# KhanhNguyen4999/Speech-Enhancement-CLSKD

Hardware: AMD Instinct MI355X
Metric: frames/sec/GPU DCCRN-CLSKD fwd+loss @16k 4s; SI-SNR parity ±0.01 dB (higher is better)
Workload: dtype bf16; 1 GPU; C2: DCCRN-CLSKD fwd+loss (teacher 3.67M + student 0.23M params, ReviewKD enc+dec, 14 SPKD Grams, MRSTFT); global_batch=16, per_gpu_batch=16, clip_samples=64000, frames_per_clip=643, parallelism=dp1, abf_reinit=step

## Files before the change

include/clskd.h:

```cpp
#ifndef CLSKD_H
#define CLSKD_H

#include <stdint.h>

#ifdef __cplusplus
extern "C" {
#endif

typedef enum {
  CLSKD_OK = 0,
  CLSKD_E_SHAPE = -1,
  CLSKD_E_DTYPE = -2,
  CLSKD_E_HIP = -3,
  CLSKD_E_ARG = -4
} clskd_status;

typedef enum { CLSKD_F32 = 0, CLSKD_BF16 = 1, CLSKD_F16 = 2, CLSKD_F32X3 = 3 } clskd_compute;

const char* clskd_last_error(void);
int clskd_version(void);

int clskd_set_knob(const char* name, int32_t value);
int clskd_get_knob(const char* name, int32_t* value);
int clskd_experiments_build(void);
// ... 43 lines not shown
  const struct clskd_bn_fold_s* bn_fold;
} clskd_conv_desc;

#define CLSKD_BN_FOLD_REPL 8
typedef struct clskd_bn_fold_s {
  int64_t* acc;
  uint32_t* ticket;
  int32_t finalize;
  int32_t C;
  int32_t c_off;
  int32_t n_updates;
  int64_t count;
  const float* gamma;
  const float* beta;
  float eps, momentum;
  float* running_mean;
  float* running_var;
  float* scale;
  float* shift;
  float* mean_out;
  float* var_out;
} clskd_bn_fold;

int64_t clskd_bn_fold_state_size(int32_t C);
int clskd_abf_bn1_fold(const float* s, int32_t B, int32_t F, int32_t T, int64_t sB, int64_t sF,
                       int64_t sT, int32_t cin, const float* w1, const clskd_bn_fold* fold,
                       int32_t nblk, void* stream);
int32_t clskd_conv_fold_capable(const clskd_conv_desc* d);

#define CLSKD_WLAYOUT_NK 0
#define CLSKD_WLAYOUT_DIRECT 1

int clskd_conv2d_fwd(const clskd_conv_desc* d, void* stream);
const char* clskd_conv_last_kernel(void);
const void* clskd_conv_last_kernel_fn(void);
int32_t clskd_conv_last_stream_k(void);
int clskd_stream_prepare(void* stream);
int clskd_capture_scope_begin(void* const* streams, int32_t nstreams, void** scope);
int clskd_capture_scope_end(void* scope);
int clskd_capture_scope_free(void* scope);
int clskd_conv_direct_np(int32_t N);
int clskd_conv_direct_ok(int32_t N, int32_t K);

int clskd_bn_stats_partial(const void* x, int64_t rows, int32_t C, double* partial,
                           int32_t nblk, int32_t dtype, void* stream);
int clskd_bn_compact(const double* partial, int32_t nblk, int32_t C, int32_t group, double* out,
                     void* stream);
int clskd_bn_finalize(double* partial, int32_t nblk, int64_t rows, int32_t C,
                      const float* gamma, const float* beta, float eps,
                      float* running_mean, float* running_var, float momentum,
                      int32_t n_updates, float* scale, float* shift, float* mean_out,
                      float* var_out, void* stream);
int clskd_bn_eval_coeffs(const float* running_mean, const float* running_var,
                         const float* gamma, const float* beta, float eps, int32_t C,
                         float* scale, float* shift, void* stream);
int clskd_bn_apply(const void* x, void* y, int64_t rows, int32_t C, const float* scale,
                   const float* shift, const float* alpha, int32_t dtype, void* stream);
int clskd_bn_apply_reim(const void* x, void* y, int64_t rows, int32_t C, const float* scale,
                        const float* shift, const float* alpha_re_im, int32_t dtype,
                        void* stream);
int32_t clskd_bn_partial_blocks(int64_t rows, int32_t C);

int clskd_lstm_recurrent(const float* gx, int64_t gx_ws, int64_t gx_seq, int64_t gx_t,
                         const float* whh, int32_t nws, int32_t nseq, int32_t T, int32_t H,
                         float* out, int64_t o_ws, int64_t o_seq, int64_t o_t, void* stream);
int clskd_lstm_pre_capable(int32_t H);
// ... 285 lines not shown
```

speech-enhancement-clskd_amd/clskd/_lib.py:

```python
import ctypes as C
import os

import torch

_HERE = os.path.dirname(os.path.abspath(__file__))
_LIB_ENV = os.environ.get("CLSKD_LIB", "")
LIB_PATH = os.path.join(_HERE, "libclskd_hip_exp.so" if _LIB_ENV == "exp"
                        else (os.path.basename(_LIB_ENV) if _LIB_ENV.endswith(".so")
                              else "libclskd_hip.so"))

MAX_SEGS = 4
F32, BF16, F16 = 0, 1, 2
F32X3 = 3
WLAYOUT_NK, WLAYOUT_DIRECT = 0, 1


class Seg(C.Structure):
    _fields_ = [("ptr", C.c_void_p), ("sB", C.c_int64), ("sF", C.c_int64), ("sT", C.c_int64),
                ("F", C.c_int32), ("T", C.c_int32)]


class KtabEntry(C.Structure):
    _fields_ = [("off", C.c_int32), ("dF", C.c_int16), ("dT", C.c_int16)]


class ConvDesc(C.Structure):
    _fields_ = [("B", C.c_int32), ("Fo", C.c_int32), ("To", C.c_int32), ("N", C.c_int32),
                ("K", C.c_int32), ("stride_f", C.c_int32), ("stride_t", C.c_int32),
                ("nseg", C.c_int32), ("seg", Seg * MAX_SEGS), ("ktab", C.c_void_p),
                ("kseg", C.c_void_p), ("vec4", C.c_int32), ("weight", C.c_void_p),
                ("bias", C.c_void_p), ("out", C.c_void_p), ("oB", C.c_int64), ("oF", C.c_int64),
                ("oT", C.c_int64), ("oNhi", C.c_int64), ("oNlo", C.c_int64), ("nlo", C.c_int32),
                ("of_mul", C.c_int32), ("of_add", C.c_int32), ("compute", C.c_int32),
                ("in_dtype", C.c_int32), ("out_dtype", C.c_int32), ("stats", C.c_void_p),
                ("kvec", C.c_int32), ("wlayout", C.c_int32), ("ntaps", C.c_int32),
                ("ctot", C.c_int32), ("seg_c", C.c_int32 * MAX_SEGS), ("tap_df", C.c_int16 * 16),
                ("tap_dt", C.c_int16 * 16), ("accumulate", C.c_int32), ("reserved_", C.c_int32),
                ("bn_fold", C.c_void_p)]


BN_FOLD_REPL = 8


class BnFold(C.Structure):
    _fields_ = [("acc", C.c_void_p), ("ticket", C.c_void_p), ("finalize", C.c_int32),
                ("C", C.c_int32), ("c_off", C.c_int32), ("n_updates", C.c_int32),
                ("count", C.c_int64), ("gamma", C.c_void_p), ("beta", C.c_void_p),
                ("eps", C.c_float), ("momentum", C.c_float), ("running_mean", C.c_void_p),
                ("running_var", C.c_void_p), ("scale", C.c_void_p), ("shift", C.c_void_p),
                ("mean_out", C.c_void_p), ("var_out", C.c_void_p)]


class GramJob(C.Structure):
    _fields_ = [("ptr", C.c_void_p), ("sB", C.c_int64), ("P", C.c_int64), ("Ctot", C.c_int32),
                ("c0", C.c_int32), ("Cs", C.c_int32), ("chunk", C.c_int32),
                ("first_slab", C.c_int32), ("nslab", C.c_int32), ("dtype", C.c_int32),
                ("reserved", C.c_int32), ("scale", C.c_void_p), ("shift", C.c_void_p),
                ("alpha", C.c_void_p), ("out", C.c_void_p)]


class DrawJob(C.Structure):
    _fields_ = [("param", C.c_void_p), ("packed", C.c_void_p), ("numel", C.c_int64),
                ("Cin", C.c_int32), ("ntap", C.c_int32), ("Kp", C.c_int32),
                ("packed_dtype", C.c_int32), ("bound", C.c_float), ("stream_id", C.c_int32)]


class GramBwdJob(C.Structure):
    _fields_ = [("ptr", C.c_void_p), ("sB", C.c_int64), ("P", C.c_int64), ("Ctot", C.c_int32),
                ("c0", C.c_int32), ("Cs", C.c_int32), ("dtype", C.c_int32), ("scale", C.c_void_p),
                ("shift", C.c_void_p), ("coef", C.c_void_p), ("out", C.c_void_p),
                ("o_sB", C.c_int64), ("o_Ctot", C.c_int32), ("o_c0", C.c_int32),
# ... 34 lines not shown


assert C.sizeof(KtabEntry) == 8
assert C.sizeof(DrawJob) == 48
assert C.sizeof(GramJob) == 88

_p, _i32, _i64, _f32 = C.c_void_p, C.c_int32, C.c_int64, C.c_float

GATHER_JOBS_MAX = 48


class GatherJob(C.Structure):
    _fields_ = [("src", C.c_void_p), ("idx", C.c_void_p), ("sgn", C.c_void_p), ("out", C.c_void_p),
                ("n", C.c_int64), ("J", C.c_int32), ("accumulate", C.c_int32)]

SIGNATURES = {
    "clskd_last_error": (C.c_char_p, []),
    "clskd_conv_last_kernel": (C.c_char_p, []),
    "clskd_conv_last_kernel_fn": (_p, []),
    "clskd_conv_last_stream_k": (_i32, []),
    "clskd_exec_launch_ahead": (_i32, [_p, _p, C.c_uint32, _p]),
    "clskd_stream_prepare": (_i32, [_p]),
    "clskd_capture_scope_begin": (_i32, [_p, _i32, _p]),
    "clskd_exec_census": (_i32, [_p, _p, _i32, _p, _p, _p]),
    "clskd_kernel_name": (_i32, [_p, _p, _i32]),
    "clskd_capture_scope_end": (_i32, [_p]),
    "clskd_capture_scope_free": (_i32, [_p]),
    "clskd_version": (_i32, []),
    "clskd_set_knob": (_i32, [C.c_char_p, _i32]),
    "clskd_get_knob": (_i32, [C.c_char_p, C.POINTER(C.c_int32)]),
    "clskd_experiments_build": (_i32, []),
    "clskd_conv2d_fwd": (_i32, [C.POINTER(ConvDesc), _p]),
    "clskd_conv_fold_capable": (_i32, [C.POINTER(ConvDesc)]),
    "clskd_bn_fold_state_size": (_i64, [_i32]),
    "clskd_abf_bn1_fold": (_i32, [_p, _i32, _i32, _i32, _i64, _i64, _i64, _i32, _p, _p, _i32, _p]),
    "clskd_conv_direct_np": (_i32, [_i32]),
    "clskd_conv_direct_ok": (_i32, [_i32, _i32]),
    "clskd_bn_partial_blocks": (_i32, [_i64, _i32]),
    "clskd_bn_stats_partial": (_i32, [_p, _i64, _i32, _p, _i32, _i32, _p]),
    "clskd_bn_compact": (_i32, [_p, _i32, _i32, _i32, _p, _p]),
    "clskd_bn_finalize": (_i32, [_p, _i32, _i64, _i32, _p, _p, _f32, _p, _p, _f32, _i32, _p, _p,
                                 _p, _p, _p]),
    "clskd_bn_eval_coeffs": (_i32, [_p, _p, _p, _p, _f32, _i32, _p, _p, _p]),
    "clskd_bn_apply": (_i32, [_p, _p, _i64, _i32, _p, _p, _p, _i32, _p]),
    "clskd_bn_apply_reim": (_i32, [_p, _p, _i64, _i32, _p, _p, _p, _i32, _p]),
    "clskd_mask_bdt": (_i32, [_p, _i32, _p, _i32, _i32, _i32, _p, _i32, _p]),
    "clskd_lstm_recurrent": (_i32, [_p, _i64, _i64, _i64, _p, _i32, _i32, _i32, _i32, _p, _i64,
                                    _i64, _i64, _p]),
    "clskd_lstm_recurrent_pre": (_i32, [_p, _i64, _i64, _i64, _p, _i32, _i32, _i32, _i32, _p, _i64,
                                        _i64, _i64, _p, _p]),
    "clskd_lstm_pre_capable": (_i32, [_i32]),
    "clskd_complex_combine": (_i32, [_p, _p, _p, _p, _p, _p, _i64, _p]),
    "clskd_complex_combine_dt": (_i32, [_p, _p, _p, _p, _p, _p, _i64, _i32, _p]),
    "clskd_lstm_cell": (_i32, [_p, _i64, _i64, _p, _i32, _i32, _i32, _p, _p, _i64, _i64, _p, _i64,
                               _i64, _p]),
    "clskd_frame_pad": (_i32, [_p, _i64, _i32, _i32, _i32, _i32, _i32, _p, _p]),
    "clskd_spec_bftc": (_i32, [_p, _i32, _i32, _i32, _i32, _i32, _i32, _p, _p]),
    "clskd_mask_e": (_i32, [_p, _i32, _p, _i32, _i32, _i32, _p, _i32, _p, _p, _p]),
    "clskd_ola": (_i32, [_p, _p, _i32, _i32, _i32, _i32, _i32, _i32, _i32, _p, _p]),
    "clskd_abf_fuse": (_i32, [_p, _p, _i32, _i32, _i32, _i32, _i32, _p, _p, _p, _p, _p, _i32,
                              _p]),
    "clskd_abf_moment_blocks": (_i32, [_i64, _i32]),
    "clskd_abf_bn1_partials": (_i32, [_p, _i32, _i32, _i32, _i64, _i64, _i64, _i32, _p, _p, _i32,
                                      _p]),
    "clskd_abf_conv1_fuse": (_i32, [_p, _i32, _i32, _i32, _i64, _i64, _i64, _i32, _p, _p, _p, _p,
                                    _i32, _i32, _p, _p, _p, _p, _i32, _p]),
# ... 150 lines not shown
```

speech-enhancement-clskd_amd/clskd/build.py:

```python
import concurrent.futures as cf
import os
import subprocess

HERE = os.path.dirname(os.path.abspath(__file__))
CSRC = os.path.join(os.path.dirname(HERE), "csrc")
OUT = os.path.join(HERE, "libclskd_hip.so")
OUT_EXP = os.path.join(HERE, "libclskd_hip_exp.so")
OBJDIR = os.path.join(os.path.dirname(HERE), "build", "obj")
OBJDIR_EXP = os.path.join(os.path.dirname(HERE), "build", "obj_exp")
HIPCC = os.environ.get("HIPCC", "/opt/rocm/bin/hipcc")
ARCH = "gfx950"
SOURCES = ["capi.cpp", "conv_igemm.hip", "conv_bf16.hip", "conv_halo.hip", "conv_halo32.hip", "conv_gemm8.hip", "conv_split.hip", "conv_direct.hip", "conv_pointwise.hip", "norm.hip", "lstm.hip", "loss.hip", "redraw.hip", "grad.hip", "wgrad_x3.hip", "norm_bwd.hip", "abf.hip", "metrics.hip", "exec.cpp", "stream_hop.hip", "stream_hop_mini.hip"]
EXPERIMENT_SOURCES = ["conv_halow.hip"]
FLAGS = ["-O3", "-fPIC", "-std=c++17", f"--offload-arch={ARCH}", "-Wall", "-Wno-unused-function"]


def _newer(src_files, target):
    if not os.path.exists(target):
        return True
    t = os.path.getmtime(target)
    return any(os.path.getmtime(s) > t for s in src_files)


def build(verbose=False, force=False, experiments=None):
    if experiments is None:
        experiments = os.environ.get("CLSKD_EXPERIMENTS") == "1"
    objdir, out = (OBJDIR_EXP, OUT_EXP) if experiments else (OBJDIR, OUT)
    flags = FLAGS + (["-DCLSKD_EXPERIMENTS"] if experiments else [])
    os.makedirs(objdir, exist_ok=True)
    headers = [os.path.join(CSRC, f) for f in os.listdir(CSRC) if f.endswith(".h")]
    headers.append(os.path.join(os.path.dirname(os.path.dirname(HERE)), "include", "clskd.h"))
    objs = []
    jobs = []
    for s in SOURCES + (EXPERIMENT_SOURCES if experiments else []):
        src = os.path.join(CSRC, s)
        obj = os.path.join(objdir, s + ".o")
        objs.append(obj)
        if force or _newer([src] + headers, obj):
            lang = ["-x", "hip"] if s.endswith(".hip") else []
            jobs.append([HIPCC] + flags + lang + ["-c", src, "-o", obj])
    with cf.ThreadPoolExecutor(max_workers=min(8, max(1, len(jobs)))) as ex:
        for cmd, res in zip(jobs, ex.map(lambda c: subprocess.run(c, capture_output=True, text=True), jobs)):
            if res.returncode != 0:
                raise RuntimeError(f"hipcc failed: {' '.join(cmd)}\n{res.stdout}\n{res.stderr}")
            if verbose and res.stderr.strip():
# ... 12 lines not shown
```

speech-enhancement-clskd_amd/csrc/capi.cpp:

```cpp
#include <stdarg.h>
#include <stdio.h>
#include <stdlib.h>

#include <atomic>
#include <mutex>

#include "common.h"

namespace clskd {
static thread_local char g_err[512] = "";
void set_error(const char* fmt, ...) {
  va_list ap;
  va_start(ap, fmt);
  vsnprintf(g_err, sizeof(g_err), fmt, ap);
  va_end(ap);
}
static thread_local char g_kernel[160] = "";
void note_kernel(const char* fmt, ...) {
  va_list ap;
  va_start(ap, fmt);
  vsnprintf(g_kernel, sizeof(g_kernel), fmt, ap);
  va_end(ap);
}

// ... 1 lines not shown
void note_kernel_fn(const void* fn) { g_kernel_fn = fn; }

struct KnobDef {
  const char* name;
  int dflt;
  bool product;
};
static const KnobDef kKnobs[KNOB_COUNT] = {
    {"CLSKD_G8", 1, false},          {"CLSKD_G8_GRID", 0, true},      {"CLSKD_HALO_GRID", 0, false},
    {"CLSKD_LSTM_NKS", 4, false},    {"CLSKD_LSTM_NKS32", 1, true},   {"CLSKD_WGRAD_WG", 4096, false},
    {"CLSKD_NO_HALO", 0, false},     {"CLSKD_BF16_WAVES", 8, false},  {"CLSKD_BF16_STAGES", 3, false},
    {"CLSKD_BF16_TILE", 0, false},   {"CLSKD_NO_POINTWISE", 0, false},
    {"CLSKD_ABF_MOMENT_DIV", 1, false}, {"CLSKD_F32_WAVES", 4, false}, {"CLSKD_EXEC_GATE", 0, false},
    {"CLSKD_NO_HALO32", 0, true},
    {"CLSKD_HALO32_SPLIT", 0, true}, {"CLSKD_HALO32_MIN_N", 32, true}, {"CLSKD_G8_KORDER", 1, false},
    {"CLSKD_G8_PP", 0, false},
    {"CLSKD_F32_SPLIT", 0, true},
    {"CLSKD_LSTM_PRIO", 0, true},
    {"CLSKD_SPLIT_BK", 0, true},
    {"CLSKD_HALOW", 0, false},
    {"CLSKD_SPLIT_GRID", 0, true},
    {"CLSKD_G8_TA", 1, true},
    {"CLSKD_G8_SK", 1, true},
    {"CLSKD_SPLIT_PD", 1, true},
    {"CLSKD_SPLIT_OCC", 1, true},
    {"CLSKD_WGRAD_DEPTH", 0, true},
    {"CLSKD_LSTM_BWD_WAVE", 1, true},
    {"CLSKD_SPLIT_NS2", 1, true},
    {"CLSKD_BN_PFOLD", 1, true},
    {"CLSKD_LSTM_PRE", 1, true},
    {"CLSKD_ABF_BWD_BLOCKS", 2048, false},
    {"CLSKD_WGRAD_XCD", 1, true},
    {"CLSKD_LSTM_BWD_PIN", 1, true},
    {"CLSKD_LSTM128_TDIV", 0, false},
    {"CLSKD_LSTM32_TDIV", 0, false}, {"CLSKD_BF16_DEBUG_MODE", 0, false}, {"CLSKD_SKIP", 0, false},
    {"CLSKD_H32_DEBUG_MODE", 0, false},
};
#ifdef CLSKD_EXPERIMENTS
static constexpr bool kAllKnobs = true;
#else
static constexpr bool kAllKnobs = false;
#endif
static std::atomic<int> g_knob[KNOB_COUNT];
static std::once_flag g_knob_once;

static void init_knobs() {
  for (int i = 0; i < KNOB_COUNT; ++i) {
    const char* e = (kAllKnobs || kKnobs[i].product) ? getenv(kKnobs[i].name) : nullptr;
    g_knob[i].store(e && *e ? atoi(e) : kKnobs[i].dflt, std::memory_order_relaxed);
  }
}

int knob(KnobId k) {
  std::call_once(g_knob_once, init_knobs);
  return g_knob[k].load(std::memory_order_relaxed);
}

static int knob_index(const char* name) {
  if (!name) return -1;
  for (int i = 0; i < KNOB_COUNT; ++i)
    if (strcmp(name, kKnobs[i].name) == 0) return i;
  return -1;
}

bool skip_kernel(int bit) {
#ifdef CLSKD_EXPERIMENTS
// ... 54 lines not shown
```

speech-enhancement-clskd_amd/csrc/common.h:

```cpp
#pragma once
#include <hip/hip_runtime.h>
#include <stdint.h>
#include <stdio.h>
#include <string.h>

#include "../../include/clskd.h"

namespace clskd {

void set_error(const char* fmt, ...);
void note_kernel(const char* fmt, ...);
void note_kernel_fn(const void* fn);
enum KnobId {
  KNOB_G8, KNOB_G8_GRID, KNOB_HALO_GRID, KNOB_LSTM_NKS, KNOB_LSTM_NKS32,
  KNOB_WGRAD_WG, KNOB_NO_HALO, KNOB_BF16_WAVES, KNOB_BF16_STAGES, KNOB_BF16_TILE,
  KNOB_NO_POINTWISE, KNOB_ABF_MOMENT_DIV, KNOB_F32_WAVES, KNOB_EXEC_GATE,
  KNOB_NO_HALO32, KNOB_HALO32_SPLIT, KNOB_HALO32_MIN_N, KNOB_G8_KORDER, KNOB_G8_PP, KNOB_F32_SPLIT, KNOB_LSTM_PRIO, KNOB_SPLIT_BK, KNOB_HALOW, KNOB_SPLIT_GRID, KNOB_G8_TA, KNOB_G8_SK, KNOB_SPLIT_PD, KNOB_SPLIT_OCC, KNOB_WGRAD_DEPTH, KNOB_LSTM_BWD_WAVE, KNOB_SPLIT_NS2, KNOB_BN_PFOLD, KNOB_LSTM_PRE, KNOB_ABF_BWD_BLOCKS, KNOB_WGRAD_XCD, KNOB_LSTM_BWD_PIN,
  KNOB_LSTM128_TDIV, KNOB_LSTM32_TDIV, KNOB_BF16_DEBUG_MODE, KNOB_SKIP, KNOB_H32_DEBUG_MODE,
  KNOB_COUNT
};
int knob(KnobId k);
int fold_partials(double* part, int nblk, int E, int bit, hipStream_t st);
int experiment_guard(const char* what, int value);
enum SkipBit {
  SKIP_BN_FINALIZE = 1, SKIP_BN_APPLY = 2, SKIP_CONV_F32 = 4, SKIP_LSTM = 8, SKIP_ABF = 16,
  SKIP_GRAM = 32, SKIP_CONV_LOWP = 64, SKIP_CONV_DIRECT = 128, SKIP_LSTM_PRE = 256, SKIP_LSTM_BWD = 512
};
bool skip_kernel(int bit);
template <typename T> inline const char* type_name();
template <> inline const char* type_name<float>() { return "float"; }
template <> inline const char* type_name<__bf16>() { return "bf16"; }
template <> inline const char* type_name<_Float16>() { return "f16"; }
template <typename T> constexpr int lowp_code() { return sizeof(T) == 4 ? CLSKD_F32 : CLSKD_BF16; }
template <> constexpr int lowp_code<_Float16>() { return CLSKD_F16; }
inline bool is_lowp(int dt) { return dt == CLSKD_BF16 || dt == CLSKD_F16; }

#define CLSKD_CHECK_ARG(cond, ...)                 \
  do {                                             \
    if (!(cond)) {                                 \
      ::clskd::set_error(__VA_ARGS__);             \
      return CLSKD_E_ARG;                          \
    }                                              \
  } while (0)

#define CLSKD_CHECK_SHAPE(cond, ...)               \
  do {                                             \
    if (!(cond)) {                                 \
      ::clskd::set_error(__VA_ARGS__);             \
      return CLSKD_E_SHAPE;                        \
    }                                              \
// ... 135 lines not shown
```

speech-enhancement-clskd_amd/csrc/conv_igemm.hip:

```cpp
#include <stdlib.h>

#include "common.h"

namespace clskd {

constexpr int BK = 16;

struct ConvArgs {
  clskd_conv_desc d;
  int kt_taps, kt_cpt;
};

__device__ __forceinline__ int swz(int row, int chunk) { return chunk ^ ((row >> 2) & 3); }

template <typename T>
__device__ __forceinline__ T sel4(int s, T a0, T a1, T a2, T a3) {
  const T lo = (s & 1) ? a1 : a0;
  const T hi = (s & 1) ? a3 : a2;
  return (s & 2) ? hi : lo;
}

template <typename OutT>
__device__ __forceinline__ void store_val(OutT* p, float v) { *p = (OutT)v; }

// ... 254 lines not shown
      d.stats[(blk * d.N + n) * 2] = S;
      d.stats[(blk * d.N + n) * 2 + 1] = Q;
    }
  }

  OutT* outp = reinterpret_cast<OutT*>(d.out);
#pragma unroll
  for (int t = 0; t < NT; ++t) {
    const int n = n0 + t * 32 + (lane & 31);
    if (n >= d.N) continue;
    const int64_t coff = (int64_t)(n / d.nlo) * d.oNhi + (int64_t)(n % d.nlo) * d.oNlo;
#pragma unroll
    for (int r = 0; r < 16; ++r) {
      const int row = wave * 32 + (r & 3) + 8 * (r >> 2) + 4 * h;
      const int64_t ro = out_row[row];
      if (ro >= 0) {
        float v = acc[t][r];
        if constexpr (sizeof(OutT) == 4) {
          if (d.accumulate) v += outp[ro + coff];
        }
        store_val<OutT>(outp + ro + coff, v);
      }
    }
  }
}

int launch_conv_bf16(const clskd_conv_desc& d, hipStream_t st);

int launch_conv_direct(const clskd_conv_desc& d, hipStream_t st);

int launch_conv_pointwise(const clskd_conv_desc& d, hipStream_t st, bool* launched);
int launch_conv_halo_f32(const clskd_conv_desc& d, hipStream_t st, bool* launched);
int launch_conv_split3(const clskd_conv_desc& d, hipStream_t st, bool* launched, bool force);

}

using namespace clskd;

namespace clskd {
bool conv_halo_takes(const clskd_conv_desc& d);
bool conv_halo_f32_takes(const clskd_conv_desc& d);
bool conv_gemm8_takes(const clskd_conv_desc& d);
#ifdef CLSKD_EXPERIMENTS
bool conv_halow_takes(const clskd_conv_desc& d);
#endif
bool conv_pointwise_takes(const clskd_conv_desc& d);
bool conv_split3_takes(const clskd_conv_desc& d, bool force);
}

static bool fold_capable(const clskd_conv_desc& dd) {
  if (dd.wlayout == CLSKD_WLAYOUT_DIRECT || dd.accumulate) return false;
  if (is_lowp(dd.compute)) {
    if (conv_halo_takes(dd)) return true;
#ifdef CLSKD_EXPERIMENTS
    if (conv_halow_takes(dd)) return true;
#endif
    return conv_gemm8_takes(dd) && dd.N <= 256;
  }
  const bool split = dd.compute == CLSKD_F32X3;
  clskd_conv_desc d = dd;
  d.compute = CLSKD_F32;
  if (conv_pointwise_takes(d)) return false;
  if (conv_split3_takes(d, split)) return true;
  return knob(KNOB_NO_HALO32) != 1 && conv_halo_f32_takes(d);
}

extern "C" int32_t clskd_conv_fold_capable(const clskd_conv_desc* dp) {
  if (!dp) return 0;
  return fold_capable(*dp) ? 1 : 0;
}

extern "C" int64_t clskd_bn_fold_state_size(int32_t C) {
  return C > 0 ? (int64_t)CLSKD_BN_FOLD_REPL * C * 6 : 0;
}

extern "C" int clskd_conv2d_fwd(const clskd_conv_desc* dp, void* stream) {
  CLSKD_CHECK_ARG(dp != nullptr, "conv2d: null descriptor");
  CLSKD_CHECK_ARG(dp->compute == CLSKD_F32 || dp->compute == CLSKD_BF16 || dp->compute == CLSKD_F16 ||
                      dp->compute == CLSKD_F32X3,
                  "conv2d: unknown compute %d", dp->compute);
  CLSKD_CHECK_ARG(dp->compute != CLSKD_F32X3 || dp->in_dtype == CLSKD_F32,
                  "conv2d: split products (CLSKD_F32X3) take fp32 segments");
  const bool want_split = dp->compute == CLSKD_F32X3;
  clskd_conv_desc dcopy = *dp;
  if (want_split) dcopy.compute = CLSKD_F32;
  const clskd_conv_desc& d = dcopy;
  CLSKD_CHECK_SHAPE(d.B > 0 && d.Fo > 0 && d.To > 0 && d.N > 0 && d.K > 0, "conv2d: empty shape");
  if (const clskd_bn_fold* f = d.bn_fold) {
    CLSKD_CHECK_ARG(!d.stats, "conv2d: bn_fold and stats are exclusive");
    CLSKD_CHECK_ARG(f->acc && f->ticket && f->scale && f->shift, "conv2d: bn_fold null pointer");
    CLSKD_CHECK_SHAPE(f->C > 0 && f->c_off >= 0 && f->c_off + d.N <= f->C && f->count > 0,
                      "conv2d: bn_fold channels [%d, +%d) outside C=%d", f->c_off, d.N, f->C);
    CLSKD_CHECK_ARG(fold_capable(*dp), "conv2d: N=%d K=%d dispatches to a kernel without the folded "
                    "BatchNorm finalize (clskd_conv_fold_capable)", d.N, d.K);
  }
// ... 27 lines not shown
  }
  const int64_t M = (int64_t)d.B * d.Fo * d.To;
  CLSKD_CHECK_SHAPE(M < (int64_t)INT32_MAX * 64, "conv2d: too many rows");
  hipStream_t st = as_stream(stream);
  CLSKD_CHECK_SHAPE(d.kvec == 0 || d.kvec == 1 || d.kvec == 2 || d.kvec == 4 || d.kvec == 8,
                    "conv2d: kvec=%d", d.kvec);
  CLSKD_CHECK_ARG(d.wlayout == CLSKD_WLAYOUT_NK || d.wlayout == CLSKD_WLAYOUT_DIRECT,
                  "conv2d: wlayout=%d", d.wlayout);
  CLSKD_CHECK_ARG(!d.accumulate || ((d.compute == CLSKD_F32 || d.compute == CLSKD_BF16) &&
                                     d.out_dtype == CLSKD_F32),
                  "conv2d: accumulate needs fp32 or bf16 compute and an fp32 output (the fp32 "
                  "engines, the direct kernel, the bf16 LDS-DMA engine)");
  if (d.wlayout == CLSKD_WLAYOUT_DIRECT) {
    if (skip_kernel(SKIP_CONV_DIRECT)) return CLSKD_OK;
    const int rc = launch_conv_direct(d, st);
    if (rc != CLSKD_OK) return rc;
    CLSKD_LAUNCH_CHECK("conv2d_direct");
    return CLSKD_OK;
  }
  if (lowp) {
    if (skip_kernel(SKIP_CONV_LOWP)) return CLSKD_OK;
    const int rc = launch_conv_bf16(d, st);
    if (rc != CLSKD_OK) return rc;
    CLSKD_LAUNCH_CHECK("conv2d_bf16");
    return CLSKD_OK;
  }
  if (skip_kernel(SKIP_CONV_F32)) return CLSKD_OK;
  {
    bool launched = false;
    const int rc = launch_conv_pointwise(d, st, &launched);
    if (rc != CLSKD_OK) return rc;
    if (launched) {
      CLSKD_LAUNCH_CHECK("conv2d_pointwise");
      return CLSKD_OK;
    }
  }
  {
    bool launched = false;
    const int rc = launch_conv_split3(d, st, &launched, want_split);
    if (rc != CLSKD_OK) return rc;
    if (launched) {
      CLSKD_LAUNCH_CHECK("conv2d_split3");
      return CLSKD_OK;
    }
  }
  if (knob(KNOB_NO_HALO32) != 1) {
    bool launched = false;
    const int rc = launch_conv_halo_f32(d, st, &launched);
    if (rc != CLSKD_OK) return rc;
    if (launched) {
      CLSKD_LAUNCH_CHECK("conv2d_halo_f32");
      return CLSKD_OK;
    }
  }
  ConvArgs a{d, 1, d.K / BK};
  if (knob(KNOB_G8_KORDER) != 0 && d.vec4 && d.ntaps > 1 && d.ctot % BK == 0 &&
      (int64_t)d.ntaps * d.ctot == d.K) {
    a.kt_taps = d.ntaps;
    a.kt_cpt = d.ctot / BK;
  }
  const size_t ctab_bytes = (size_t)(d.K / 4) * 8;
  CLSKD_CHECK_SHAPE(!d.vec4 || ctab_bytes <= 32 * 1024, "conv2d(f32): K=%d too long for the chunk table", d.K);
  const int nw = knob(KNOB_F32_WAVES) == 8 ? 8 : 4;
#define LAUNCH(BN_, V_, O_, NW_)                                                             \
  do {                                                                                       \
    hipLaunchKernelGGL((conv_igemm_f32<BN_, V_, O_, NW_>),                                    \
// ... 28 lines not shown
```

Measured before the change: 2.007 million frames/s.

## Add halo-tiled split-bf16 (3-pass) MFMA conv kernel for F32X3 convolutions

```diff
diff --git a/include/clskd.h b/include/clskd.h
--- a/include/clskd.h
+++ b/include/clskd.h
@@ -99,6 +99,21 @@
 #define CLSKD_WLAYOUT_DIRECT 1
 
 int clskd_conv2d_fwd(const clskd_conv_desc* d, void* stream);
+
+typedef struct {
+  int32_t launches, col_halves;
+  int32_t cw;
+  int32_t tile_f, tile_t;
+  int32_t nfb, ntb, ntiles;
+  int32_t halo_f, halo_t;
+  int32_t nchunk, nstep;
+  int32_t grid;
+  int32_t reserved_;
+  int64_t lds_bytes;
+  int64_t seg_min_off[CLSKD_MAX_SEGS];
+  int64_t seg_max_off[CLSKD_MAX_SEGS];
+} clskd_halo_split_info;
+int clskd_conv_halo_split_plan(const clskd_conv_desc* d, clskd_halo_split_info* info);
 const char* clskd_conv_last_kernel(void);
 const void* clskd_conv_last_kernel_fn(void);
 int32_t clskd_conv_last_stream_k(void);
diff --git a/speech-enhancement-clskd_amd/clskd/_lib.py b/speech-enhancement-clskd_amd/clskd/_lib.py
--- a/speech-enhancement-clskd_amd/clskd/_lib.py
+++ b/speech-enhancement-clskd_amd/clskd/_lib.py
@@ -37,6 +37,15 @@
                 ("ctot", C.c_int32), ("seg_c", C.c_int32 * MAX_SEGS), ("tap_df", C.c_int16 * 16),
                 ("tap_dt", C.c_int16 * 16), ("accumulate", C.c_int32), ("reserved_", C.c_int32),
                 ("bn_fold", C.c_void_p)]
+
+
+class HaloSplitInfo(C.Structure):
+    _fields_ = [("launches", C.c_int32), ("col_halves", C.c_int32), ("cw", C.c_int32), ("tile_f", C.c_int32),
+                ("tile_t", C.c_int32), ("nfb", C.c_int32), ("ntb", C.c_int32),
+                ("ntiles", C.c_int32), ("halo_f", C.c_int32), ("halo_t", C.c_int32),
+                ("nchunk", C.c_int32), ("nstep", C.c_int32), ("grid", C.c_int32), ("reserved_", C.c_int32),
+                ("lds_bytes", C.c_int64), ("seg_min_off", C.c_int64 * MAX_SEGS),
+                ("seg_max_off", C.c_int64 * MAX_SEGS)]
 
 
 BN_FOLD_REPL = 8
@@ -137,6 +146,7 @@
     "clskd_experiments_build": (_i32, []),
     "clskd_conv2d_fwd": (_i32, [C.POINTER(ConvDesc), _p]),
     "clskd_conv_fold_capable": (_i32, [C.POINTER(ConvDesc)]),
+    "clskd_conv_halo_split_plan": (_i32, [C.POINTER(ConvDesc), C.POINTER(HaloSplitInfo)]),
     "clskd_bn_fold_state_size": (_i64, [_i32]),
     "clskd_abf_bn1_fold": (_i32, [_p, _i32, _i32, _i32, _i64, _i64, _i64, _i32, _p, _p, _i32, _p]),
     "clskd_conv_direct_np": (_i32, [_i32]),
diff --git a/speech-enhancement-clskd_amd/clskd/build.py b/speech-enhancement-clskd_amd/clskd/build.py
--- a/speech-enhancement-clskd_amd/clskd/build.py
+++ b/speech-enhancement-clskd_amd/clskd/build.py
@@ -10,7 +10,7 @@
 OBJDIR_EXP = os.path.join(os.path.dirname(HERE), "build", "obj_exp")
 HIPCC = os.environ.get("HIPCC", "/opt/rocm/bin/hipcc")
 ARCH = "gfx950"
-SOURCES = ["capi.cpp", "conv_igemm.hip", "conv_bf16.hip", "conv_halo.hip", "conv_halo32.hip", "conv_gemm8.hip", "conv_split.hip", "conv_direct.hip", "conv_pointwise.hip", "norm.hip", "lstm.hip", "loss.hip", "redraw.hip", "grad.hip", "wgrad_x3.hip", "norm_bwd.hip", "abf.hip", "metrics.hip", "exec.cpp", "stream_hop.hip", "stream_hop_mini.hip"]
+SOURCES = ["capi.cpp", "conv_igemm.hip", "conv_bf16.hip", "conv_halo.hip", "conv_halo32.hip", "conv_gemm8.hip", "conv_split.hip", "conv_halo_split.hip", "conv_direct.hip", "conv_pointwise.hip", "norm.hip", "lstm.hip", "loss.hip", "redraw.hip", "grad.hip", "wgrad_x3.hip", "norm_bwd.hip", "abf.hip", "metrics.hip", "exec.cpp", "stream_hop.hip", "stream_hop_mini.hip"]
 EXPERIMENT_SOURCES = ["conv_halow.hip"]
 FLAGS = ["-O3", "-fPIC", "-std=c++17", f"--offload-arch={ARCH}", "-Wall", "-Wno-unused-function"]
 
diff --git a/speech-enhancement-clskd_amd/csrc/capi.cpp b/speech-enhancement-clskd_amd/csrc/capi.cpp
--- a/speech-enhancement-clskd_amd/csrc/capi.cpp
+++ b/speech-enhancement-clskd_amd/csrc/capi.cpp
@@ -57,6 +57,8 @@
     {"CLSKD_ABF_BWD_BLOCKS", 2048, false},
     {"CLSKD_WGRAD_XCD", 1, true},
     {"CLSKD_LSTM_BWD_PIN", 1, true},
+    {"CLSKD_HALO_SPLIT", 1, true},
+    {"CLSKD_HALO_SPLIT_GRID", 0, true},
     {"CLSKD_LSTM128_TDIV", 0, false},
     {"CLSKD_LSTM32_TDIV", 0, false}, {"CLSKD_BF16_DEBUG_MODE", 0, false}, {"CLSKD_SKIP", 0, false},
     {"CLSKD_H32_DEBUG_MODE", 0, false},
diff --git a/speech-enhancement-clskd_amd/csrc/common.h b/speech-enhancement-clskd_amd/csrc/common.h
--- a/speech-enhancement-clskd_amd/csrc/common.h
+++ b/speech-enhancement-clskd_amd/csrc/common.h
@@ -16,6 +16,7 @@
   KNOB_WGRAD_WG, KNOB_NO_HALO, KNOB_BF16_WAVES, KNOB_BF16_STAGES, KNOB_BF16_TILE,
   KNOB_NO_POINTWISE, KNOB_ABF_MOMENT_DIV, KNOB_F32_WAVES, KNOB_EXEC_GATE,
   KNOB_NO_HALO32, KNOB_HALO32_SPLIT, KNOB_HALO32_MIN_N, KNOB_G8_KORDER, KNOB_G8_PP, KNOB_F32_SPLIT, KNOB_LSTM_PRIO, KNOB_SPLIT_BK, KNOB_HALOW, KNOB_SPLIT_GRID, KNOB_G8_TA, KNOB_G8_SK, KNOB_SPLIT_PD, KNOB_SPLIT_OCC, KNOB_WGRAD_DEPTH, KNOB_LSTM_BWD_WAVE, KNOB_SPLIT_NS2, KNOB_BN_PFOLD, KNOB_LSTM_PRE, KNOB_ABF_BWD_BLOCKS, KNOB_WGRAD_XCD, KNOB_LSTM_BWD_PIN,
+  KNOB_HALO_SPLIT, KNOB_HALO_SPLIT_GRID,
   KNOB_LSTM128_TDIV, KNOB_LSTM32_TDIV, KNOB_BF16_DEBUG_MODE, KNOB_SKIP, KNOB_H32_DEBUG_MODE,
   KNOB_COUNT
 };
diff --git a/speech-enhancement-clskd_amd/csrc/conv_halo_split.hip b/speech-enhancement-clskd_amd/csrc/conv_halo_split.hip
--- /dev/null
+++ b/speech-enhancement-clskd_amd/csrc/conv_halo_split.hip
@@ -0,0 +1,580 @@
+#include <stdlib.h>
+
+#include "bnfold.h"
+#include "common.h"
+
+namespace clskd {
+
+__device__ __attribute__((aligned(256))) unsigned char g_hs3_sink[4096];
+
+typedef __attribute__((address_space(1))) float gfloat_hs3;
+
+namespace hs3 {
+typedef short s16x8 __attribute__((ext_vector_type(8)));
+typedef short s16x4 __attribute__((ext_vector_type(4)));
+constexpr int NW = 8;
+constexpr int NTH = NW * 64;
+constexpr int MAXU = 6;
+constexpr int MAXCH = 64;
+constexpr int MAXSTEP = 16;
+
+__device__ __forceinline__ void split4(const f32x4 v, s16x4& hi, s16x4& lo) {
+  bf16x4 h, l;
+#pragma unroll
+  for (int i = 0; i < 4; ++i) {
+    h[i] = (__bf16)v[i];
+    l[i] = (__bf16)(v[i] - (float)h[i]);
+  }
+  hi = __builtin_bit_cast(s16x4, h);
+  lo = __builtin_bit_cast(s16x4, l);
+}
+
+__host__ __device__ inline int plane_off(int cw, int p, int q) {
+  return cw == 16 ? p * 32 + ((((q >> 1) ^ (p >> 3)) & 1) << 4) + (q & 1) * 8 : p * 16 + (q & 1) * 8;
+}
+}
+
+struct HaloSplitArgs {
+  clskd_conv_desc d;
+  int32_t nchunk;
+  int32_t chunk_seg[hs3::MAXCH];
+  int32_t chunk_c0[hs3::MAXCH];
+  int32_t chunk_kofs[hs3::MAXCH];
+  int32_t cw, tw;
+  int32_t dfmin, dtmin;
+  int32_t HF, HT, NPIX;
+  int32_t NU;
+  int32_t plane_bytes;
+  int32_t nstep;
+  int32_t step_pix[2][hs3::MAXSTEP];
+  int32_t step_oct[2][hs3::MAXSTEP];
+  int32_t koct;
+  int32_t nfb, ntb, ntiles;
+  int32_t nblk128;
+  int32_t stats_ld;
+  int32_t nhalf;
+  BnFoldArgs f;
+};
+
+template <int NB, int CW, int NSTEP>
+__global__ __launch_bounds__(512) void conv_halo_split3_kernel(const HaloSplitArgs a) {
+  using namespace hs3;
+  const clskd_conv_desc& d = a.d;
+  constexpr int NBW = NB * 32;
+  constexpr int QP = CW / 4;
+  constexpr int NACC = NB == 1 ? 3 : 1;
+  extern __shared__ __attribute__((aligned(16))) unsigned char smem[];
+  const int plane_bytes = a.plane_bytes;
+  unsigned char* hbuf = smem;
+  unsigned char* wl = smem + 4 * plane_bytes;
+  const int wplane = (a.koct + 1) * NBW * 16;
+  int4* ctA = reinterpret_cast<int4*>(wl + 2 * wplane);
+  int4* ctB = ctA + MAXCH;
+
+  const int tid = threadIdx.x;
+  const int lane = tid & 63;
+  const int wave = __builtin_amdgcn_readfirstlane(tid >> 6);
+  const int l32 = lane & 31, h = lane >> 5;
+  const int nhalf = a.nhalf;
+  const int half = nhalf == 2 ? (int)(blockIdx.x & 1) : 0;
+  const int wgi = blockIdx.x / nhalf, nwg = gridDim.x / nhalf;
+  const int n0 = half * 32;
+  const int N = nhalf == 2 ? min(32, d.N - n0) : d.N;
+
+  {
+    const int64_t K = d.K;
+    const float* wg = reinterpret_cast<const float*>(d.weight) + n0 * K;
+    const int total = a.koct * NBW * 2;
+    constexpr int WB = 8;
+    const int kq2 = a.koct * 2;
+    for (int base = tid; base < total; base += NTH * WB) {
+      f32x4 v[WB];
+#pragma unroll
+      for (int j = 0; j < WB; ++j) {
+        const int idx = base + j * NTH;
+        const int n = idx / kq2, kq = idx - n * kq2;
+        v[j] = (idx < total && n < N) ? *reinterpret_cast<const f32x4*>(wg + n * K + kq * 4)
+                                      : f32x4{0.f, 0.f, 0.f, 0.f};
+      }
+#pragma unroll
+      for (int j = 0; j < WB; ++j) {
+        const int idx = base + j * NTH;
+        if (idx < total) {
+          const int n = idx / kq2, kq = idx - n * kq2;
+          s16x4 hi, lo;
+          split4(v[j], hi, lo);
+          const int off = ((kq >> 1) * NBW + n) * 16 + (kq & 1) * 8;
+          *reinterpret_cast<s16x4*>(wl + off) = hi;
+          *reinterpret_cast<s16x4*>(wl + wplane + off) = lo;
+        }
+      }
+    }
+    for (int i = tid; i < NBW * 4; i += NTH) {
+      const int pl = i / (NBW * 2), piece = i - pl * NBW * 2;
+      *reinterpret_cast<int2*>(wl + pl * wplane + a.koct * NBW * 16 + piece * 8) = make_int2(0, 0);
+    }
+  }
+  if (tid < a.nchunk) {
+    const clskd_seg& S = d.seg[a.chunk_seg[tid]];
+    const uint64_t base = (uint64_t)(uintptr_t)(S.ptr + a.chunk_c0[tid]);
+    ctA[tid] = make_int4((int)(unsigned)base, (int)(unsigned)(base >> 32), (int)S.sF, (int)S.sT);
+    ctB[tid] = make_int4((int)S.sB, S.F, S.T, a.chunk_kofs[tid]);
+  }
+  if (d.stats) {
+    for (int64_t s = (int64_t)blockIdx.x + gridDim.x; s < a.nblk128; s += gridDim.x)
+      for (int i = tid; i < d.N * 2; i += NTH) d.stats[s * a.stats_ld * 2 + i] = 0.0;
+    if (nhalf == 2)
+      for (int i = tid; i < (d.N - N) * 2; i += NTH)
+        d.stats[((int64_t)blockIdx.x * a.stats_ld + (half ? 0 : 32)) * 2 + i] = 0.0;
+  }
+  float bcol[NB];
+  int64_t coff[NB];
+#pragma unroll
+  for (int nb = 0; nb < NB; ++nb) {
+    const int n = nb * 32 + l32;
+    const int ng = n0 + n;
+    bcol[nb] = (d.bias && n < N) ? d.bias[ng] : 0.f;
+    coff[nb] = n < N ? (int64_t)(ng / d.nlo) * d.oNhi + (int64_t)(ng % d.nlo) * d.oNlo : -1;
+  }
+  const int nchunk = a.nchunk, ntb = a.ntb, nfb = a.nfb, NU = a.NU;
+  const int tw = a.tw, FT = NW / tw, TT = 32 * tw;
+  const int Fo = d.Fo, To = d.To, sfr = d.stride_f;
+  const int dfmin = a.dfmin, dtmin = a.dtmin;
+  const int64_t oB = d.oB, oF = d.oF, oT = d.oT;
+  const int of_mul = d.of_mul, of_add = d.of_add;
+  gfloat_hs3* const outp = reinterpret_cast<gfloat_hs3*>((uintptr_t)d.out);
+  int ug[MAXU], uo[MAXU];
+  {
+    const int HT = a.HT, NPIX = a.NPIX;
+#pragma unroll
+    for (int i = 0; i < MAXU; ++i) {
+      const int u = tid + i * NTH;
+      const int p = u / QP, q = u % QP;
+      const bool ok = i < NU && p < NPIX;
+      const int pp = ok ? p : 0;
+      const int hf = pp / HT, ht = pp - hf * HT;
+      ug[i] = hf | (ht << 8) | (q << 16) | ((ok ? 1 : 0) << 20);
+      uo[i] = plane_off(CW, pp, q);
+    }
+  }
+  const int frow = wave / tw, tblk = wave - frow * tw;
+  int sa[NSTEP];
+  unsigned sb[NSTEP];
+  {
+    const int prow0 = frow * sfr * a.HT + tblk * 32 + l32;
+#pragma unroll
+    for (int s = 0; s < NSTEP; ++s) {
+      const int p = prow0 + (h ? a.step_pix[1][s] : a.step_pix[0][s]);
+      const int oct = h ? a.step_oct[1][s] : a.step_oct[0][s];
+      sa[s] = CW == 16 ? p * 32 + (((h ^ (p >> 3)) & 1) << 4) : p * 16;
+      sb[s] = oct < 0 ? (0x80000000u | (unsigned)((a.koct * NBW + l32) * 16))
+                      : (unsigned)((oct * NBW + l32) * 16);
+    }
+  }
+  __syncthreads();
+
+  const int per = (a.ntiles + nwg - 1) / nwg;
+  const int tile_begin = wgi * per;
+  const int ntile_blk = max(0, min(a.ntiles, tile_begin + per) - tile_begin);
+
+  struct Cur { int b, fb, tb; };
+  auto cur_of = [&](int tile) {
+    Cur c;
+    c.tb = tile % ntb;
+    const int r = tile / ntb;
+    c.fb = r % nfb;
+    c.b = r / nfb;
+    return c;
+  };
+  auto advance = [&](Cur& c) {
+    if (++c.tb == ntb) {
+      c.tb = 0;
+      if (++c.fb == nfb) { c.fb = 0; ++c.b; }
+    }
+  };
+
+  f32x4 ra[MAXU];
+  auto load_chunk = [&](const Cur& c, int ch) {
+    const int4 ea = ctA[ch];
+    const int4 eb = ctB[ch];
+    const float* base = reinterpret_cast<const float*>(((uint64_t)(unsigned)ea.y << 32) | (unsigned)ea.x) +
+                        (int64_t)c.b * eb.x;
+    const int fi_lo = c.fb * FT * sfr + dfmin, ti_lo = c.tb * TT + dtmin;
+#pragma unroll
+    for (int i = 0; i < MAXU; ++i) {
+      if (i < NU) {
+        const int g = ug[i];
+        const int fi = fi_lo + (g & 0xff), ti = ti_lo + ((g >> 8) & 0xff);
+        f32x4 v = {0.f, 0.f, 0.f, 0.f};
+        if (((g >> 20) & 1) && (unsigned)fi < (unsigned)eb.y && (unsigned)ti < (unsigned)eb.z)
+          v = *reinterpret_cast<const f32x4*>(base + (int64_t)fi * ea.z + (int64_t)ti * ea.w +
+                                              ((g >> 16) & 3) * 4);
+        ra[i] = v;
+      }
+    }
+  };
+  auto store_chunk = [&](int buf) {
+    unsigned char* hb = hbuf + buf * 2 * plane_bytes;
+#pragma unroll
+    for (int i = 0; i < MAXU; ++i) {
+      if (i < NU && ((ug[i] >> 20) & 1)) {
+        s16x4 hi, lo;
+        split4(ra[i], hi, lo);
+        *reinterpret_cast<s16x4*>(hb + uo[i]) = hi;
+        *reinterpret_cast<s16x4*>(hb + plane_bytes + uo[i]) = lo;
+      }
+    }
+  };
+
+  f32x16 acc[NACC][NB];
+  double st_s[NB], st_q[NB];
+#pragma unroll
+  for (int nb = 0; nb < NB; ++nb) st_s[nb] = st_q[nb] = 0.0;
+
+  const int total = ntile_blk * nchunk;
+  Cur cur = cur_of(tile_begin), nxt = cur;
+  int nxt_ch = 0;
+  auto step_next = [&]() {
+    if (++nxt_ch == nchunk) { nxt_ch = 0; advance(nxt); }
+  };
+  if (total > 0) {
+    load_chunk(nxt, nxt_ch);
+    step_next();
+    store_chunk(0);
+    if (total > 1) {
+      load_chunk(nxt, nxt_ch);
+      step_next();
+    }
+  }
+  __syncthreads();
+
+  int it = 0;
+  for (int ti = 0; ti < ntile_blk; ++ti) {
+#pragma unroll
+    for (int q = 0; q < NACC; ++q)
+#pragma unroll
+      for (int nb = 0; nb < NB; ++nb)
+#pragma unroll
+        for (int r = 0; r < 16; ++r) acc[q][nb][r] = q == 0 ? bcol[nb] : 0.f;
+    for (int ch = 0; ch < nchunk; ++ch, ++it) {
+      const unsigned char* hb = hbuf + (it & 1) * 2 * plane_bytes;
+      const unsigned kofsb = (unsigned)((ctB[ch].w >> 3) * NBW * 16);
+#pragma unroll
+      for (int s = 0; s < NSTEP; ++s) {
+        const s16x8 ahi = *reinterpret_cast<const s16x8*>(hb + sa[s]);
+        const s16x8 alo = *reinterpret_cast<const s16x8*>(hb + plane_bytes + sa[s]);
+        const unsigned bo = (sb[s] & 0x7fffffffu) + ((sb[s] >> 31) ? 0u : kofsb);
+        s16x8 bhi[NB], blo[NB];
+#pragma unroll
+        for (int nb = 0; nb < NB; ++nb) {
+          bhi[nb] = *reinterpret_cast<const s16x8*>(wl + bo + nb * 512);
+          blo[nb] = *reinterpret_cast<const s16x8*>(wl + wplane + bo + nb * 512);
+        }
+        if constexpr (NB == 1) {
+          acc[0][0] = mfma16<__bf16>(ahi, bhi[0], acc[0][0]);
+          acc[1][0] = mfma16<__bf16>(alo, bhi[0], acc[1][0]);
+          acc[2][0] = mfma16<__bf16>(ahi, blo[0], acc[2][0]);
+        } else {
+#pragma unroll
+          for (int nb = 0; nb < NB; ++nb) acc[0][nb] = mfma16<__bf16>(ahi, bhi[nb], acc[0][nb]);
+#pragma unroll
+          for (int nb = 0; nb < NB; ++nb) acc[0][nb] = mfma16<__bf16>(alo, bhi[nb], acc[0][nb]);
+#pragma unroll
+          for (int nb = 0; nb < NB; ++nb) acc[0][nb] = mfma16<__bf16>(ahi, blo[nb], acc[0][nb]);
+        }
+      }
+      if (it + 1 < total) store_chunk((it + 1) & 1);
+      if (it + 2 < total) {
+        load_chunk(nxt, nxt_ch);
+        step_next();
+      }
+      __syncthreads();
+    }
+    const int fo = cur.fb * FT + frow;
+    const int to0 = cur.tb * TT + tblk * 32;
+    const int64_t obase = (int64_t)cur.b * oB + (int64_t)(fo * of_mul + of_add) * oF + (int64_t)to0 * oT;
+    gfloat_hs3* sink = reinterpret_cast<gfloat_hs3*>((uintptr_t)g_hs3_sink) + lane;
+#pragma unroll
+    for (int nb = 0; nb < NB; ++nb) {
+      const bool nok = coff[nb] >= 0;
+      float sm = 0.f, sq = 0.f;
+#pragma unroll
+      for (int r = 0; r < 16; ++r) {
+        const int row = (r & 3) + 8 * (r >> 2) + 4 * h;
+        const bool ok = nok && fo < Fo && to0 + row < To;
+        float v = acc[0][nb][r];
+#pragma unroll
+        for (int q = 1; q < NACC; ++q) v += acc[q][nb][r];
+        if (ok) {
+          sm += v;
+          sq = fmaf(v, v, sq);
+        }
+        gfloat_hs3* dst = ok ? outp + obase + (int64_t)row * oT + coff[nb] : sink;
+        *dst = v;
+      }
+      st_s[nb] += (double)sm;
+      st_q[nb] += (double)sq;
+    }
+    advance(cur);
+  }
+
+  if (d.stats || a.f.acc) {
+    __syncthreads();
+    double* red = reinterpret_cast<double*>(smem);
+#pragma unroll
+    for (int nb = 0; nb < NB; ++nb) {
+      const double s2 = st_s[nb] + __shfl_xor(st_s[nb], 32, 64);
+      const double q2 = st_q[nb] + __shfl_xor(st_q[nb], 32, 64);
+      if (h == 0) {
+        red[(wave * NBW + nb * 32 + l32) * 2] = s2;
+        red[(wave * NBW + nb * 32 + l32) * 2 + 1] = q2;
+      }
+    }
+    __syncthreads();
+    auto sum_waves = [&](int n, double& S, double& Q) {
+      S = 0.0;
+      Q = 0.0;
+      for (int w = 0; w < NW; ++w) {
+        S += red[(w * NBW + n) * 2];
+        Q += red[(w * NBW + n) * 2 + 1];
+      }
+    };
+    if (a.f.acc) {
+      BnFoldArgs f = a.f;
+      f.c_off += n0;
+      bnfold_commit(f, N, sum_waves, reinterpret_cast<int*>(red + NW * NBW * 2), blockIdx.x,
+                    gridDim.x);
+    } else if (blockIdx.x < a.nblk128) {
+      for (int n = tid; n < N; n += NTH) {
+        double S, Q;
+        sum_waves(n, S, Q);
+        d.stats[((int64_t)blockIdx.x * a.stats_ld + n0 + n) * 2] = S;
+        d.stats[((int64_t)blockIdx.x * a.stats_ld + n0 + n) * 2 + 1] = Q;
+      }
+    }
+  }
+}
+
+static bool halo_split_plan1(const clskd_conv_desc& d, HaloSplitArgs& a, size_t& lds, int cw) {
+  using namespace hs3;
+  if (d.in_dtype != CLSKD_F32 || d.compute != CLSKD_F32 || d.out_dtype != CLSKD_F32) return false;
+  if (d.accumulate || d.wlayout != CLSKD_WLAYOUT_NK) return false;
+  if (d.N < 16 || d.N > 64 || d.ntaps < 1 || d.ntaps > 16 || d.stride_t != 1) return false;
+  if (d.stride_f < 1 || d.stride_f > 2 || d.ctot < cw || d.ctot % cw) return false;
+  if (d.nseg < 1 || d.nseg > CLSKD_MAX_SEGS) return false;
+  a.d = d;
+  a.cw = cw;
+  int nch = 0, kofs = 0;
+  for (int s = 0; s < d.nseg; ++s) {
+    const clskd_seg& g = d.seg[s];
+    if (d.seg_c[s] < cw || d.seg_c[s] % cw) return false;
+    if (((uintptr_t)g.ptr & 15) || g.sB % 4 || g.sF % 4 || g.sT % 4) return false;
+    if (g.sB < 0 || g.sF < 0 || g.sT < 0) return false;
+    if (g.sB > INT32_MAX || g.sF > INT32_MAX || g.sT > INT32_MAX) return false;
+    for (int c0 = 0; c0 < d.seg_c[s]; c0 += cw) {
+      if (nch >= MAXCH) return false;
+      a.chunk_seg[nch] = s;
+      a.chunk_c0[nch] = c0;
+      a.chunk_kofs[nch] = kofs + c0;
+      ++nch;
+    }
+    kofs += d.seg_c[s];
+  }
+  if (kofs != d.ctot || d.ntaps * d.ctot > d.K || d.K % 8) return false;
+  if (((uintptr_t)d.weight & 15)) return false;
+  a.nchunk = nch;
+  int dfmin = 1 << 20, dfmax = -(1 << 20), dtmin = 1 << 20, dtmax = -(1 << 20);
+  for (int t = 0; t < d.ntaps; ++t) {
+    dfmin = d.tap_df[t] < dfmin ? d.tap_df[t] : dfmin;
+    dfmax = d.tap_df[t] > dfmax ? d.tap_df[t] : dfmax;
+    dtmin = d.tap_dt[t] < dtmin ? d.tap_dt[t] : dtmin;
+    dtmax = d.tap_dt[t] > dtmax ? d.tap_dt[t] : dtmax;
+  }
+  a.tw = d.Fo <= 4 ? 2 : 1;
+  const int FT = NW / a.tw, TT = 32 * a.tw;
+  a.dfmin = dfmin;
+  a.dtmin = dtmin;
+  a.HF = (FT - 1) * d.stride_f + (dfmax - dfmin + 1);
+  a.HT = (TT - 1) + (dtmax - dtmin + 1);
+  if (a.HF > 255 || a.HT > 255) return false;
+  a.NPIX = a.HF * a.HT;
+  a.NU = (int)cdiv((int64_t)a.NPIX * (cw / 4), NTH);
+  if (a.NU > MAXU) return false;
+  a.plane_bytes = (a.NPIX * cw * 2 + 15) & ~15;
+  a.koct = d.ntaps * d.ctot / 8;
+  a.nstep = cw == 16 ? d.ntaps : (d.ntaps + 1) / 2;
+  if (a.nstep > MAXSTEP) return false;
+  for (int h = 0; h < 2; ++h)
+    for (int s = 0; s < MAXSTEP; ++s) {
+      const int t = cw == 16 ? s : 2 * s + h;
+      const bool on = s < a.nstep && t < d.ntaps;
+      a.step_pix[h][s] = on ? (d.tap_df[t] - dfmin) * a.HT + (d.tap_dt[t] - dtmin) : 0;
+      a.step_oct[h][s] = on ? t * (d.ctot / 8) + (cw == 16 ? h : 0) : -1;
+    }
+  const int NBW = d.N <= 32 ? 32 : 64;
+  lds = 4 * (size_t)a.plane_bytes + 2 * (size_t)(a.koct + 1) * NBW * 16 + 2 * MAXCH * 16;
+  if (lds > 160 * 1024) return false;
+  if ((size_t)NW * NBW * 16 + 16 > 4 * (size_t)a.plane_bytes) return false;
+  a.nfb = (int)cdiv(d.Fo, FT);
+  a.ntb = (int)cdiv(d.To, TT);
+  const int64_t nt = (int64_t)d.B * a.nfb * a.ntb;
+  if (nt < 32 || nt > (1 << 30)) return false;
+  a.ntiles = (int)nt;
+  a.nblk128 = (int)cdiv((int64_t)d.B * d.Fo * d.To, 128);
+  a.stats_ld = d.N;
+  a.nhalf = 1;
+  a.f = make_bnfold(d);
+  return true;
+}
+
+static bool halo_split_plan(const clskd_conv_desc& d, HaloSplitArgs& a, size_t& lds) {
+  return halo_split_plan1(d, a, lds, 16) || halo_split_plan1(d, a, lds, 8);
+}
+
+static bool halo_split_plans(const clskd_conv_desc& d, HaloSplitArgs& a, size_t& lds) {
+  if (knob(KNOB_HALO_SPLIT) != 1) return false;
+  if (halo_split_plan(d, a, lds)) return true;
+  if (d.N <= 32 || d.N > 64) return false;
+  clskd_conv_desc d1 = d, d2 = d;
+  d1.N = 32;
+  d2.N = d.N - 32;
+  HaloSplitArgs a2;
+  size_t lds2 = 0;
+  if (!halo_split_plan(d2, a2, lds2) || !halo_split_plan(d1, a, lds)) return false;
+  if (a2.cw != a.cw || lds2 != lds) return false;
+  a.d = d;
+  a.stats_ld = d.N;
+  a.nhalf = 2;
+  return true;
+}
+
+static int halo_split_grid(const HaloSplitArgs& a) {
+  static int ncu = [] {
+    int v = 256;
+    (void)hipDeviceGetAttribute(&v, hipDeviceAttributeMultiprocessorCount, 0);
+    return v > 0 ? v : 256;
+  }();
+  const int gcap = knob(KNOB_SPLIT_GRID);
+  int cus = gcap > 0 && gcap < ncu ? gcap : ncu;
+  const int own = knob(KNOB_HALO_SPLIT_GRID);
+  if (own > 0 && own < cus) cus = own;
+  int nwg = cus / a.nhalf;
+  nwg = a.ntiles < nwg ? a.ntiles : nwg;
+  if (a.d.stats && nwg * a.nhalf > a.nblk128) nwg = a.nblk128 / a.nhalf;
+  return (nwg > 0 ? nwg : 1) * a.nhalf;
+}
+
+static bool halo_split_built(const HaloSplitArgs& a) {
+  const int n = a.nstep;
+  return a.cw == 16 ? (n == 4 || n == 6 || n == 9 || n == 10) : (n == 2 || n == 3 || n == 5);
+}
+
+static void launch_halo_split_planned(const HaloSplitArgs& a, size_t lds, hipStream_t st) {
+  const int grid = halo_split_grid(a);
+#define HS3_LAUNCH(NB_, CW_, NS_)                                                              \
+  do {                                                                                         \
+    auto k = conv_halo_split3_kernel<NB_, CW_, NS_>;                                           \
+    (void)hipFuncSetAttribute((const void*)k, hipFuncAttributeMaxDynamicSharedMemorySize,      \
+                              160 * 1024);                                                     \
+    hipLaunchKernelGGL(k, dim3(grid), dim3(512), lds, st, a);                                  \
+    note_kernel_fn((const void*)k);                                                            \
+    note_kernel("conv_halo_split3_kernel<%d,%d,%d>", NB_, CW_, NS_);                           \
+  } while (0)
+#define HS3_NB(CW_, NS_)                                                                       \
+  do {                                                                                         \
+    if (a.d.N <= 32 || a.nhalf == 2) HS3_LAUNCH(1, CW_, NS_); else HS3_LAUNCH(2, CW_, NS_);                    \
+  } while (0)
+  if (a.cw == 16) {
+    switch (a.nstep) {
+      case 4: HS3_NB(16, 4); break;
+      case 6: HS3_NB(16, 6); break;
+      case 9: HS3_NB(16, 9); break;
+      default: HS3_NB(16, 10); break;
+    }
+  } else {
+    switch (a.nstep) {
+      case 2: HS3_NB(8, 2); break;
+      case 3: HS3_NB(8, 3); break;
+      default: HS3_NB(8, 5); break;
+    }
+  }
+#undef HS3_NB
+#undef HS3_LAUNCH
+}
+
+static bool halo_split_taken(const clskd_conv_desc& d, HaloSplitArgs& a, size_t& lds) {
+  return halo_split_plans(d, a, lds) && halo_split_built(a);
+}
+
+bool conv_halo_split_takes(const clskd_conv_desc& d) {
+  HaloSplitArgs a;
+  size_t lds = 0;
+  return halo_split_taken(d, a, lds);
+}
+
+int launch_conv_halo_split(const clskd_conv_desc& d, hipStream_t st, bool* launched) {
+  HaloSplitArgs a;
+  size_t lds = 0;
+  *launched = halo_split_taken(d, a, lds);
+  if (*launched) launch_halo_split_planned(a, lds, st);
+  return CLSKD_OK;
+}
+
+}
+
+extern "C" int clskd_conv_halo_split_plan(const clskd_conv_desc* dp, clskd_halo_split_info* info) {
+  using namespace clskd;
+  using namespace clskd::hs3;
+  CLSKD_CHECK_ARG(dp && info, "halo_split_plan: null argument");
+  memset(info, 0, sizeof(*info));
+  clskd_conv_desc d = *dp;
+  if (d.compute == CLSKD_F32X3) d.compute = CLSKD_F32;
+  HaloSplitArgs a;
+  size_t lds = 0;
+  if (!halo_split_taken(d, a, lds)) return CLSKD_OK;
+  info->launches = 1;
+  info->col_halves = a.nhalf;
+  for (int s = 0; s < CLSKD_MAX_SEGS; ++s) {
+    info->seg_min_off[s] = INT64_MAX;
+    info->seg_max_off[s] = INT64_MIN;
+  }
+  {
+    const HaloSplitArgs& p = a;
+    info->cw = p.cw;
+    info->tile_f = NW / p.tw;
+    info->tile_t = 32 * p.tw;
+    info->nfb = p.nfb;
+    info->ntb = p.ntb;
+    info->ntiles = p.ntiles;
+    info->halo_f = p.HF;
+    info->halo_t = p.HT;
+    info->nchunk = p.nchunk;
+    info->nstep = p.nstep;
+    info->lds_bytes = (int64_t)lds;
+    info->grid = halo_split_grid(p);
+    const int QP = p.cw / 4, FT = NW / p.tw, TT = 32 * p.tw;
+    for (int s = 0; s < p.nstep; ++s)
+      for (int h = 0; h < 2; ++h) {
+        const int pmax = (FT - 1) * p.d.stride_f * p.HT + (p.tw - 1) * 32 + 31 + p.step_pix[h][s];
+        CLSKD_CHECK_ARG(pmax < p.NPIX, "halo_split_plan: fragment pixel %d outside the halo %d", pmax, p.NPIX);
+      }
+    for (int tile = 0; tile < p.ntiles; ++tile) {
+      const int tb = tile % p.ntb, fb = (tile / p.ntb) % p.nfb, b = tile / p.ntb / p.nfb;
+      const int fi_lo = fb * FT * p.d.stride_f + p.dfmin, ti_lo = tb * TT + p.dtmin;
+      for (int ch = 0; ch < p.nchunk; ++ch) {
+        const int sg = p.chunk_seg[ch];
+        const clskd_seg& S = p.d.seg[sg];
+        for (int u = 0; u < p.NU * NTH; ++u) {
+          const int px = u / QP, q = u % QP;
+          if (px >= p.NPIX) continue;
+          const int fi = fi_lo + px / p.HT, ti = ti_lo + px % p.HT;
+          if ((unsigned)fi >= (unsigned)S.F || (unsigned)ti >= (unsigned)S.T) continue;
+          const int64_t off = p.chunk_c0[ch] + (int64_t)b * S.sB + (int64_t)fi * S.sF + (int64_t)ti * S.sT + q * 4;
+          if (off < info->seg_min_off[sg]) info->seg_min_off[sg] = off;
+          if (off + 3 > info->seg_max_off[sg]) info->seg_max_off[sg] = off + 3;
+        }
+      }
+    }
+  }
+  return CLSKD_OK;
+}
diff --git a/speech-enhancement-clskd_amd/csrc/conv_igemm.hip b/speech-enhancement-clskd_amd/csrc/conv_igemm.hip
--- a/speech-enhancement-clskd_amd/csrc/conv_igemm.hip
+++ b/speech-enhancement-clskd_amd/csrc/conv_igemm.hip
@@ -310,6 +310,7 @@
 int launch_conv_pointwise(const clskd_conv_desc& d, hipStream_t st, bool* launched);
 int launch_conv_halo_f32(const clskd_conv_desc& d, hipStream_t st, bool* launched);
 int launch_conv_split3(const clskd_conv_desc& d, hipStream_t st, bool* launched, bool force);
+int launch_conv_halo_split(const clskd_conv_desc& d, hipStream_t st, bool* launched);
 
 }
 
@@ -324,6 +325,7 @@
 #endif
 bool conv_pointwise_takes(const clskd_conv_desc& d);
 bool conv_split3_takes(const clskd_conv_desc& d, bool force);
+bool conv_halo_split_takes(const clskd_conv_desc& d);
 }
 
 static bool fold_capable(const clskd_conv_desc& dd) {
@@ -339,6 +341,7 @@
   clskd_conv_desc d = dd;
   d.compute = CLSKD_F32;
   if (conv_pointwise_takes(d)) return false;
+  if (split && conv_halo_split_takes(d)) return true;
   if (conv_split3_takes(d, split)) return true;
   return knob(KNOB_NO_HALO32) != 1 && conv_halo_f32_takes(d);
 }
@@ -432,6 +435,15 @@
     if (rc != CLSKD_OK) return rc;
     if (launched) {
       CLSKD_LAUNCH_CHECK("conv2d_pointwise");
+      return CLSKD_OK;
+    }
+  }
+  if (want_split) {
+    bool launched = false;
+    const int rc = launch_conv_halo_split(d, st, &launched);
+    if (rc != CLSKD_OK) return rc;
+    if (launched) {
+      CLSKD_LAUNCH_CHECK("conv2d_halo_split");
       return CLSKD_OK;
     }
   }
```

After: 2.052 million frames/s, median of 6. 2.3% higher.
